# EspressoSystems/Push-CDN

Measured on AMD Instinct MI355X. Metric: broadcast_msgs_per_sec, higher is better.
Workload: dtype uint8; 1 GPU; model=gpu-broker-mesh, payload_bytes=1024, subscribers_total=10000, subscribers_per_broker=10000, topics=8, mode=broadcast, population=all, drops=0, parallelism=single-broker, global_batch=256, seq_len=1024

## Files before the change

csrc/common/tick_geom.h:

```cpp
#pragma once

#include <stdint.h>

#define K2B_BLK 32

#define DENSE_THREADS 256
#define DENSE_MAX_V 8
#define DENSE_GROUP 8
struct DenseGeom { int32_t n_chunks; int32_t chunk_units; };
static inline DenseGeom dense_geom(int32_t units_per_rec) {
    const int32_t cap = DENSE_THREADS * DENSE_MAX_V;
    const int32_t image = units_per_rec * K2B_BLK;
    DenseGeom g;
    g.n_chunks = (image + cap - 1) / cap;
    g.chunk_units = ((image + g.n_chunks - 1) / g.n_chunks + 63) & ~63;
    return g;
}
static inline int64_t dense_grid_x(int32_t n_users, int32_t group, int32_t n_chunks) {
    return ((int64_t)n_users + group - 1) / group * n_chunks;
}

static inline int64_t k2b_blocks(int64_t M) { return (M + K2B_BLK - 1) / K2B_BLK; }
static inline int64_t uniform_tick_scratch64(int64_t M, int64_t W, int64_t units_per_rec) {
    return 4 * M + W * M + k2b_blocks(M) * W * 64 + W * 64 + 2 * M * units_per_rec;
}
static inline int64_t uniform_tick_scratch32(int64_t M, int64_t W) {
    return 3 * M + 3 * k2b_blocks(M) * W * 64 + 2 * W * 64;
}

#define ROUTE_THREADS 256
struct RouteLds { int32_t mask, udst, ulim, usbase, pprefix, tslot, bcount, bytes; };
constexpr RouteLds route_lds(int32_t M) {
    const int32_t tiles = (M + K2B_BLK - 1) / K2B_BLK * 64;
    RouteLds l{};
    l.mask = 0;
    l.udst = l.mask + 8 * M;
    l.ulim = l.udst + 8 * 64;
    l.usbase = l.ulim + 4 * 64;
    l.pprefix = l.usbase + 4 * 64;
    l.tslot = l.pprefix + 2 * tiles;
    l.bcount = l.tslot + 2 * tiles;
    l.bytes = l.bcount + tiles;
    return l;
}
#define ROUTE_MAX_M 3584
static_assert(route_lds(ROUTE_MAX_M).bytes <= 64 * 1024, "route kernel LDS exceeds a workgroup's 64 KiB");
static_assert(route_lds(ROUTE_MAX_M + 1).bytes > 64 * 1024, "ROUTE_MAX_M is not the largest batch that fits");
static_assert(ROUTE_MAX_M >= 2048, "the 8-GPU bench routes 8 x 256 gathered messages per tick");
static_assert(ROUTE_MAX_M <= 65535 && K2B_BLK <= 255, "prefixes are 16-bit, tile counts 8-bit");
static_assert(route_lds(33).udst % 8 == 0 && route_lds(33).ulim % 4 == 0 && route_lds(33).pprefix % 2 == 0,
              "route kernel LDS arrays are aligned to their element types");
```

csrc/gpu_bindings.cpp:

```cpp

#include "binding_checks.h"
#include "hip/bls_kernels.h"
#include "hip/dataplane.h"

static inline void check_flat_shape(const torch::Tensor& pairs, int64_t units_per_pair) {
    TORCH_CHECK(units_per_pair >= 1 && units_per_pair <= (int64_t(1) << 21),
                "units_per_pair must be in [1, 2^21], got ", units_per_pair);
    TORCH_CHECK(pairs.size(0) * units_per_pair < (int64_t(1) << 31),
                "pair capacity * units_per_pair must be < 2^31, got ", pairs.size(0), " * ",
                units_per_pair);
}

std::vector<torch::Tensor> parse_batch(torch::Tensor buf, torch::Tensor offsets,
                                       uint64_t hash_seed) {
    Op a("parse_batch");
    const uint8_t* b = a.ptr<uint8_t>(buf, "buf");
    const int64_t* off = a.ptr<int64_t>(offsets, "offsets", 1);
    const int32_t M = a.i32(offsets.numel() - 1, "M");
    hipStream_t s = a.begin();
    auto o32 = opts(torch::kInt32, buf);
    auto o64 = opts(torch::kInt64, buf);
    auto disc = torch::empty({M}, o32);
    auto payload_off = torch::empty({M}, o64);
    auto payload_len = torch::empty({M}, o32);
// ... 485 lines not shown
}

void emit_direct_peers(torch::Tensor disc, torch::Tensor owner, torch::Tensor origin,
                       torch::Tensor payload_off, torch::Tensor payload_len,
                       int64_t ring_bytes, int64_t n_users, int64_t n_peers,
                       torch::Tensor ring_wpos, torch::Tensor n_pairs, torch::Tensor pairs,
                       torch::Tensor drops) {
    Op a("emit_direct_peers");
    const DirectArgs d = direct_args(a, disc, owner, payload_off, payload_len, ring_bytes);
    const int32_t* org = a.same<int32_t>(origin, "origin", d.M, "one per disc");
    const int32_t n = a.i32(n_users, "n_users");
    const int32_t p = a.i32(n_peers, "n_peers");
    uint64_t* wpos = a.ptr<uint64_t>(ring_wpos, "ring_wpos", int64_t(n) + p);
    int32_t* np = a.ptr<int32_t>(n_pairs, "n_pairs", 1);
    PairRec* pr = a.pairs(pairs);
    const int32_t capacity = a.i32(pairs.size(0), "pair capacity");
    uint32_t* dr = a.ptr<uint32_t>(drops, "drops", 1);
    hipStream_t s = a.begin();
    if (d.M == 0) return;
    launch_k5b_emit_direct_peers(d.disc, d.owner, org, d.payload_off, d.payload_len, d.M, n, p,
                                 ring_bytes, capacity, wpos, np, pr, dr, s);
    a.launched();
}

void direct_apply(torch::Tensor table_keys, torch::Tensor table_vals, torch::Tensor up_keys,
                  torch::Tensor up_owners, torch::Tensor del_keys, torch::Tensor n_failed) {
    Op a("direct_apply");
    uint64_t* keys = a.ptr<uint64_t>(table_keys, "table_keys", 1, vec());
    const int64_t S = table_keys.numel();
    TORCH_CHECK((S & (S - 1)) == 0, a.name(), ": table_keys must have a power-of-two length, got ",
                S);
    int32_t* vals = a.same<int32_t>(table_vals, "table_vals", S, "one per table_keys");
    const uint64_t* up = a.ptr<uint64_t>(up_keys, "up_keys");
    const int32_t n_up = a.i32(up_keys.numel(), "upsert count");
    const int32_t* owners = a.same<int32_t>(up_owners, "up_owners", n_up, "one per up_keys");
    const uint64_t* del = a.ptr<uint64_t>(del_keys, "del_keys");
    const int32_t n_del = a.i32(del_keys.numel(), "delete count");
    uint32_t* failed = a.ptr<uint32_t>(n_failed, "n_failed", 1);
    hipStream_t s = a.begin();
    launch_k6_direct_apply(keys, vals, S, up, owners, n_up, del, n_del, failed, s);
    a.launched();
}

void tick_uniform_broadcast(torch::Tensor buf, torch::Tensor offsets, uint64_t hash_seed,
                            torch::Tensor sub_bitmap, torch::Tensor ring_wpos,
                            int64_t ring_bytes, int64_t n_users, torch::Tensor pairs,
                            torch::Tensor drops, torch::Tensor n_pairs, torch::Tensor n_sparse,
                            torch::Tensor scratch64, torch::Tensor scratch32,
                            int64_t uniform_len, int64_t seq_base, torch::Tensor egress,
                            int64_t nt, int64_t dense) {
    Op a("tick_uniform_broadcast");
    UniformTick t;
    t.uniform_len = a.i32(uniform_len, "uniform_len", 0, (int64_t(1) << 30) - 1);
    const int64_t rec = (uniform_len + 16 + 15) & ~int64_t(15);
    t.rec = a.i32(rec, "rec");
    t.buf = a.ptr<uint8_t>(buf, "buf");
    t.offsets = a.ptr<int64_t>(offsets, "offsets", 1);
    const int64_t M = offsets.numel() - 1;
    t.M = a.i32(M, "M");
    t.hash_seed = hash_seed;
    t.sub_bitmap = a.ptr<uint64_t>(sub_bitmap, "sub_bitmap", 0, mat(256, -1));
    const int64_t W = sub_bitmap.size(1);
    t.W = a.i32(W, "W");
    t.n_users = a.i32(n_users, "n_users", 0, W * 64);
    a.ring_bytes(ring_bytes);
    t.ring_bytes = ring_bytes;
    t.ring_wpos = a.ptr<uint64_t>(ring_wpos, "ring_wpos", n_users);
    t.pairs = a.pairs(pairs);
    t.capacity = a.i32(pairs.size(0), "pair capacity");
    t.drops = a.ptr<uint32_t>(drops, "drops", 1);
    t.n_pairs = a.ptr<int32_t>(n_pairs, "n_pairs", 1);
    t.n_sparse = a.ptr<int32_t>(n_sparse, "n_sparse", 1);
    t.scratch64 = a.ptr<int64_t>(scratch64, "scratch64", uniform_tick_scratch64(M, W, rec / 16));
    t.scratch32 = a.ptr<int32_t>(scratch32, "scratch32", uniform_tick_scratch32(M, W));
    t.egress = a.ptr<uint8_t>(egress, "egress", n_users * ring_bytes);
    t.seq_base = (uint32_t)seq_base;
    t.nt = nt != 0;
    t.dense = dense != 0;
    TORCH_CHECK(buf.numel() >= M * uniform_len, a.name(), ": buf has ", buf.numel(),
                " bytes, shorter than M = ", M, " messages of uniform_len = ", uniform_len);
    check_flat_shape(pairs, rec / 16);
    TORCH_CHECK(M * (rec / 16) < (int64_t(1) << 31)
                && dense_grid_x(t.n_users, DENSE_GROUP, dense_geom((int32_t)(rec / 16)).n_chunks)
                       * k2b_blocks(M) < (int64_t(1) << 31),
                a.name(), ": batch too large for the dense fan-out");
    TORCH_CHECK((uintptr_t)t.scratch64 % 16 == 0, a.name(), ": scratch64 must be 16-byte aligned");
    hipStream_t s = a.begin();
    if (M == 0) return;
    launch_tick_uniform_broadcast(&t, s);
    a.launched();
}

std::vector<int64_t> uniform_tick_scratch_sizes(int64_t M, int64_t W, int64_t rec) {
    return {uniform_tick_scratch64(M, W, rec / 16), uniform_tick_scratch32(M, W)};
}

void drain_cursors(torch::Tensor ring_wpos, torch::Tensor staging, torch::Tensor host) {
    Op a("drain_cursors");
    int64_t* wpos = a.ptr<int64_t>(ring_wpos, "ring_wpos");
    const int32_t n = a.i32(ring_wpos.numel(), "cursor count");
    int64_t* st = a.ptr<int64_t>(staging, "staging", n);
    int64_t* h = a.ptr<int64_t>(host, "host", n, {}, Op::kPinnedHost);
    hipStream_t s = a.begin();
    if (n == 0) return;
    launch_drain_cursors(wpos, st, n, s);
    a.launched();
    a.check(hipMemcpyAsync(h, st, (size_t)n * 8, hipMemcpyDeviceToHost, s), "copy");
    a.check(hipStreamSynchronize(s), "sync");
}

PYBIND11_MODULE(TORCH_EXTENSION_NAME, m) {
    m.attr("_ROUTE_MAX_M") = py::int_(ROUTE_MAX_M);
    m.def("tick_uniform_broadcast", &tick_uniform_broadcast,
          "fused uniform broadcast tick: K4, K2a, K2b tiles, dense + sparse fan-out");
    m.def("uniform_tick_scratch_sizes", &uniform_tick_scratch_sizes,
          "(int64, int32) scratch elements tick_uniform_broadcast needs for (M, W, rec)");
    m.def("drain_cursors", &drain_cursors,
          "fused drain: cursors -> pinned host buffer, cursors zeroed, stream synchronised",
          py::call_guard<py::gil_scoped_release>());
    m.def("topic_mask_origin_t", &topic_mask_origin_t,
          "K2a transposed with per-message origin: remote-origin rows keep user bits only");
    m.def("emit_direct_peers", &emit_direct_peers,
          "K5b with peer recipient slots (owner -(p+2) -> ring n_users+p, local origin only)");
    m.def("direct_apply", &direct_apply,
          "K6: batched DirectMap upserts/deletes on the device table");
    m.def("parse_batch", &parse_batch, "K4: on-device capnp parse of a message batch",
          py::arg("buf"), py::arg("offsets"), py::arg("hash_seed") = 0);
    m.def("topic_mask", &topic_mask, "K2a: per-message subscriber mask");
    m.def("assign_emit", &assign_emit, "K2b: per-user FIFO ring assignment + pair list");
    m.def("fanout", &fanout, "K3: N-way payload fan-out into egress rings");
    m.def("direct_lookup", &direct_lookup, "K5: batched direct-route hash probe");
    m.def("apply_subs", &apply_subs, "K2c: apply subscribe/unsubscribe batch to bitmap");
    m.def("bls_verify_batch", &bls_verify_batch, "K1: batched BLS-over-BN254 verification");
    m.def("compact_rings", &compact_rings,
          "K7: gather used egress-ring prefixes into one staging buffer");
    m.def("precompute_g2_lines", &precompute_g2_lines,
          "fixed-g2 Miller line coefficients for K1 v2 (once per process)");
    m.def("bls_verify_batch2", &bls_verify_batch2,
          "K1 v2: 2-lane Fp2-decomposed batched BLS verification");
    m.def("bls_verify_batch_wave", &bls_verify_batch_wave,
          "K1 v3: wave-batched product verification (shared final exp, "
          "exact per-item fallback)");
    m.def("hash_to_g1_batch", &hash_to_g1_batch, "K1 helper: batched hash-to-G1");
    m.def("fanout_wave", &fanout_wave, "K3v2: wave-per-pair fan-out (nt flag, device count)");
    m.def("fanout_ref", &fanout_ref,
          "K3r: fan-out with by-reference records at or above ref_threshold");
    m.def("fanout_flat2", &fanout_flat2, "K3v4: flat fan-out, seq from base, capacity clamp");
    m.def("fanout_flat3", &fanout_flat3, "K3v5: graph-capturable (device seq counter)");
    m.def("seq_advance", &seq_advance, "bump the device seq counter (inside the graph)");
    m.def("topic_mask_t", &topic_mask_t, "K2a transposed: mask[W][M]");
    m.def("emit_direct", &emit_direct,
          "K5b: on-device direct-delivery pair emission (no host sync)");
    m.def("assign_emit_fused_t", &assign_emit_fused_t,
          "K2b fused on transposed mask (wave-aggregated claims, uniform-rec fast path)");
    m.def("assign_emit_blocks_t", &assign_emit_blocks_t,
          "K2b block-parallel (P1 count / P2 bases / P3 emit) for uniform records");
}
```

csrc/hip/dataplane.h:

```cpp
#pragma once

#include <hip/hip_runtime_api.h>
#include <stdint.h>

#include "../common/tick_geom.h"

struct alignas(16) PairRec { int32_t user; int32_t msg; int64_t dst; };
static_assert(sizeof(PairRec) == 16, "PairRec must be one dword4");

struct ParseOut {
    int32_t* disc;
    int64_t* payload_off;
    int32_t* payload_len;
    int64_t* topics_off;
    int32_t* topics_cnt;
    uint64_t* recip_hash;
    uint64_t* timestamp;
};

struct UniformTick {
    const uint8_t* buf;
    const int64_t* offsets;
    int32_t M;
    uint64_t hash_seed;
// ... 19 lines not shown

extern "C" {

void launch_k4_parse(const uint8_t* buf, const int64_t* offsets, int32_t M, uint64_t hash_seed,
                     ParseOut out, hipStream_t s);

void launch_k2a_topic_mask(const uint64_t* sub_bitmap, const uint8_t* buf,
                           const int64_t* topics_off, const int32_t* topics_cnt,
                           const int32_t* disc, uint64_t* mask, int32_t M, int32_t W,
                           hipStream_t s);
void launch_k2a_topic_mask_t(const uint64_t* sub_bitmap, const uint8_t* buf,
                             const int64_t* topics_off, const int32_t* topics_cnt,
                             const int32_t* disc, uint64_t* mask_t, int32_t M, int32_t W,
                             hipStream_t s);
void launch_k2a_topic_mask_origin_t(const uint64_t* sub_bitmap, const uint8_t* buf,
                                    const int64_t* topics_off, const int32_t* topics_cnt,
                                    const int32_t* disc, const int32_t* origin,
                                    uint64_t* mask_t, int32_t M, int32_t W, int32_t n_users,
                                    hipStream_t s);
void launch_k2c_apply_subs(uint64_t* sub_bitmap, const uint8_t* buf, const int64_t* topics_off,
                           const int32_t* topics_cnt, const int32_t* disc,
                           const int32_t* user_idx, int32_t M, int32_t W, hipStream_t s);

void launch_k2b_count(const uint64_t* mask, int32_t M, int32_t W, int32_t n_users,
                      int32_t* counts, hipStream_t s);
void launch_k2b_emit(const uint64_t* mask, const int64_t* payload_off,
                     const int32_t* payload_len, const int32_t* pair_base, int32_t M, int32_t W,
                     int32_t n_users, int64_t ring_bytes, uint64_t* ring_wpos, PairRec* pairs,
                     uint32_t* drops, hipStream_t s);
void launch_k2b_fused_t(const uint64_t* mask_t, const int32_t* payload_len, int32_t M,
                        int32_t W, int32_t n_users, int64_t ring_bytes, int32_t capacity,
                        int32_t uniform_rec, uint64_t* ring_wpos, int32_t* n_pairs,
                        PairRec* pairs, uint32_t* drops, hipStream_t s);
void launch_k2b_blocks_t(const uint64_t* mask_t, int32_t M, int32_t W, int32_t n_users,
                         int64_t ring_bytes, int32_t capacity, int32_t uniform_rec,
                         uint64_t* ring_wpos, int32_t* n_pairs, int32_t* bcount,
                         int32_t* pprefix, int32_t* ubase, int32_t* ufit, int64_t* udst,
                         PairRec* pairs, uint32_t* drops, hipStream_t s);

void launch_k3_fanout(const uint8_t* buf, const int64_t* payload_off,
                      const int32_t* payload_len, const PairRec* pairs, const uint32_t* msg_seq,
                      int32_t n_pairs, uint8_t* egress, hipStream_t s);
void launch_k3_fanout_wave(const uint8_t* buf, const int64_t* payload_off,
                           const int32_t* payload_len, const PairRec* pairs,
                           const uint32_t* msg_seq, const int32_t* n_pairs_ptr,
                           int32_t capacity, uint8_t* egress, int nt, int grid, hipStream_t s);
void launch_k3_fanout_ref(const uint8_t* buf, const int64_t* payload_off,
                          const int32_t* payload_len, const PairRec* pairs,
                          const uint32_t* msg_seq, const int32_t* n_pairs_ptr,
                          int32_t capacity, int32_t ref_threshold, int64_t ref_base,
                          uint8_t* egress, int nt, int grid, hipStream_t s);
void launch_k3_fanout_flat2(const uint8_t* buf, const int64_t* payload_off,
                            const int32_t* payload_len, const PairRec* pairs,
                            uint32_t seq_base, const int32_t* n_pairs_ptr, int32_t capacity,
                            int32_t units_per_pair, int32_t uniform_len, uint8_t* egress,
                            int nt, int grid, hipStream_t s);
void launch_k3_fanout_flat3(const uint8_t* buf, const int64_t* payload_off,
                            const int32_t* payload_len, const PairRec* pairs,
                            const uint32_t* seq_state, const int32_t* n_pairs_ptr,
                            int32_t capacity, int32_t units_per_pair, int32_t uniform_len,
                            uint8_t* egress, int nt, int grid, hipStream_t s);
void launch_k_seq_advance(uint32_t* seq_state, int32_t m, hipStream_t s);

void launch_k5_direct_lookup(const uint64_t* table_keys, const int32_t* table_vals,
                             int64_t table_size, const uint64_t* query, int32_t N,
                             int32_t* owner, hipStream_t s);
void launch_k5b_emit_direct(const int32_t* disc, const int32_t* owner,
                            const int64_t* payload_off, const int32_t* payload_len, int32_t M,
                            int64_t ring_bytes, int32_t capacity, uint64_t* ring_wpos,
                            int32_t* n_pairs, PairRec* pairs, uint32_t* drops, hipStream_t s);
void launch_k5b_emit_direct_peers(const int32_t* disc, const int32_t* owner,
                                  const int32_t* origin, const int64_t* payload_off,
                                  const int32_t* payload_len, int32_t M, int32_t n_users,
                                  int32_t n_peers, int64_t ring_bytes, int32_t capacity,
                                  uint64_t* ring_wpos, int32_t* n_pairs, PairRec* pairs,
                                  uint32_t* drops, hipStream_t s);
void launch_k6_direct_apply(uint64_t* table_keys, int32_t* table_vals, int64_t table_size,
                            const uint64_t* up_keys, const int32_t* up_owners, int32_t n_up,
                            const uint64_t* del_keys, int32_t n_del, uint32_t* n_failed,
                            hipStream_t s);

void launch_tick_uniform_broadcast(const UniformTick* t, hipStream_t s);

void launch_drain_cursors(int64_t* ring_wpos, int64_t* staging, int32_t n, hipStream_t s);

void launch_k7_compact_rings(const uint8_t* egress, int64_t ring_bytes, const int64_t* wpos,
                             const int64_t* dst_off, uint8_t* staging, int32_t n_rings,
                             int32_t max_chunks, hipStream_t s);

}
```

csrc/hip/dataplane.hip:

```cpp

#include <hip/hip_runtime.h>
#include <stdint.h>

#include "../common/divmagic.h"
#include "dataplane.h"

#define WAVE 64
#ifndef CDN_CHECK
#define CDN_CHECK 1
#endif

#define RING_ALIGN 16ull
__host__ __device__ inline uint64_t ring_rec(int32_t len) {
    return ((uint64_t)len + 16 + (RING_ALIGN - 1)) & ~(RING_ALIGN - 1);
}

typedef unsigned int cdn_v4u __attribute__((ext_vector_type(4)));
template <int NT>
__device__ __forceinline__ void store16(void* dst, cdn_v4u v) {
    if (NT) __builtin_nontemporal_store(v, (cdn_v4u*)dst);
    else *(cdn_v4u*)dst = v;
}

__device__ __forceinline__ void store_pair(PairRec* p, int32_t u, int32_t m, int64_t d) {
// ... 472 lines not shown
    const int64_t* __restrict__ payload_off,
    const int32_t* __restrict__ payload_len,
    const PairRec* __restrict__ pairs,
    const uint32_t* __restrict__ msg_seq,
    const int32_t* __restrict__ n_pairs_ptr,
    int32_t capacity,
    int32_t ref_threshold,
    int64_t ref_base,
    uint8_t* __restrict__ egress)
{
    int n_pairs = *n_pairs_ptr;
    if (n_pairs > capacity) n_pairs = capacity;
    const int lane = threadIdx.x & 63;
    const int wave_in_wg = threadIdx.x >> 6;
    const int waves_total = gridDim.x * 4;
    int gs = 0;
    while (gs < 6 && ((n_pairs - 1) >> gs) + 1 > waves_total) ++gs;
    const int n_groups = n_pairs > 0 ? ((n_pairs - 1) >> gs) + 1 : 0;
    for (int g = blockIdx.x * 4 + wave_in_wg; g < n_groups; g += waves_total) {
        const int64_t p = ((int64_t)g << gs) + lane;
        int32_t len = 0;
        uint32_t seq = 0;
        int64_t off = 0, dsto = 0;
        bool live = false;
        if (lane < (1 << gs) && p < n_pairs) {
            const PairRec pr = pairs[p];
            if (pr.user >= 0) {
                live = true;
                len = payload_len[pr.msg];
                off = payload_off[pr.msg];
                seq = msg_seq[pr.msg];
                dsto = pr.dst;
            }
        }
        const bool by_ref = live && len >= ref_threshold;
        if (by_ref) {
            const uint64_t ro = (uint64_t)(ref_base + off);
            store16<NT>(egress + dsto, cdn_v4u{(uint32_t)len | REF_FLAG, seq, (uint32_t)ro,
                                               (uint32_t)(ro >> 32)});
        }
        unsigned long long inl = __ballot(live && !by_ref);
        while (inl) {
            const int j = __ffsll((long long)inl) - 1;
            inl &= inl - 1;
            const int32_t jlen = __shfl(len, j);
            const uint32_t jseq = (uint32_t)__shfl((int)seq, j);
            const int64_t joff = ((int64_t)__shfl((int)(off >> 32), j) << 32)
                                 | (uint32_t)__shfl((int)off, j);
            const int64_t jdst = ((int64_t)__shfl((int)(dsto >> 32), j) << 32)
                                 | (uint32_t)__shfl((int)dsto, j);
            copy_record<NT>(egress + jdst, buf + joff, jlen, jseq, lane, WAVE);
        }
    }
}

extern "C" {

void launch_k3_fanout_ref(const uint8_t* buf, const int64_t* payload_off,
                          const int32_t* payload_len, const PairRec* pairs,
                          const uint32_t* msg_seq, const int32_t* n_pairs_ptr,
                          int32_t capacity, int32_t ref_threshold, int64_t ref_base,
                          uint8_t* egress, int nt, int grid, hipStream_t s) {
    if (grid <= 0) grid = 4096;
    DISPATCH_NT(nt, hipLaunchKernelGGL((k3_fanout_ref_t<NT>), dim3(grid), dim3(256), 0, s, buf,
                                       payload_off, payload_len, pairs, msg_seq, n_pairs_ptr,
                                       capacity, ref_threshold, ref_base, egress));
}

}

__device__ __forceinline__ cdn_v4u payload_unit(const uint8_t* __restrict__ msg, int32_t coff,
                                                int32_t len)
{
    const uint8_t* src = msg + coff;
    if (coff + 16 <= len && (((uintptr_t)src) & 15) == 0) return *(const cdn_v4u*)src;
    if (coff >= len) return cdn_v4u{0u, 0u, 0u, 0u};
    uint8_t tmp[16];
    #pragma unroll
    for (int b = 0; b < 16; ++b) tmp[b] = (coff + b < len) ? src[b] : 0;
    cdn_v4u v; memcpy(&v, tmp, 16);
    return v;
}

template <int NT, bool SEQ_FROM_PTR>
__global__ void __launch_bounds__(256) k3_fanout_flat_t(
    const uint8_t* __restrict__ buf,
    const int64_t* __restrict__ payload_off,
    const int32_t* __restrict__ payload_len,
    const PairRec* __restrict__ pairs,
    uint32_t seq_base_val,
    const uint32_t* __restrict__ seq_state,
    const int32_t* __restrict__ n_pairs_ptr,
    int32_t capacity,
    int32_t units_per_pair,
    uint32_t div_magic,
    int32_t div_shift,
    int32_t uniform_len,
    uint8_t* __restrict__ egress)
{
    const uint32_t seq_base = SEQ_FROM_PTR ? seq_state[0] : seq_base_val;
    int np = *n_pairs_ptr;
    if (np > capacity) np = capacity;
    const int64_t n_units = (int64_t)np * units_per_pair;
    const int64_t stride = (int64_t)gridDim.x * blockDim.x;
    for (int64_t f = (int64_t)blockIdx.x * blockDim.x + threadIdx.x; f < n_units; f += stride) {
        const uint32_t f32 = (uint32_t)f;
        const int p = (int)(((uint64_t)f32 * div_magic) >> div_shift);
        const int unit = (int)(f32 - (uint32_t)p * (uint32_t)units_per_pair);
        const PairRec pr = pairs[p];
        if (pr.user < 0) continue;
        const int mi = pr.msg;
        const int32_t len = uniform_len > 0 ? uniform_len : payload_len[mi];
        uint8_t* dst = egress + pr.dst + (size_t)unit * 16;
        if (unit == 0) {
            store16<NT>(dst, cdn_v4u{(uint32_t)len, seq_base + (uint32_t)mi, 0u, 0u});
            continue;
        }
        store16<NT>(dst, payload_unit(buf + payload_off[mi], (unit - 1) * 16, len));
    }
}


template <bool SEQ_FROM_PTR>
static void launch_flat(const uint8_t* buf, const int64_t* payload_off,
                        const int32_t* payload_len, const PairRec* pairs, uint32_t seq_base,
                        const uint32_t* seq_state, const int32_t* n_pairs_ptr, int32_t capacity,
                        int32_t units_per_pair, int32_t uniform_len, uint8_t* egress, int nt,
                        int grid, hipStream_t s) {
    if (grid <= 0) grid = 16384;
    uint32_t dm; int32_t dsh;
    u32_div_magic(units_per_pair, &dm, &dsh);
    DISPATCH_NT(nt, hipLaunchKernelGGL((k3_fanout_flat_t<NT, SEQ_FROM_PTR>), dim3(grid),
                                       dim3(256), 0, s, buf, payload_off, payload_len, pairs,
                                       seq_base, seq_state, n_pairs_ptr, capacity,
                                       units_per_pair, dm, dsh, uniform_len, egress));
}

extern "C" __global__ void k_seq_advance(uint32_t* seq_state, int32_t m) {
    if (blockIdx.x == 0 && threadIdx.x == 0) seq_state[0] += (uint32_t)m;
}

extern "C" {

void launch_k3_fanout_flat2(const uint8_t* buf, const int64_t* payload_off,
                            const int32_t* payload_len, const PairRec* pairs,
                            uint32_t seq_base, const int32_t* n_pairs_ptr, int32_t capacity,
                            int32_t units_per_pair, int32_t uniform_len, uint8_t* egress,
                            int nt, int grid, hipStream_t s) {
    launch_flat<false>(buf, payload_off, payload_len, pairs, seq_base, nullptr, n_pairs_ptr,
                       capacity, units_per_pair, uniform_len, egress, nt, grid, s);
}

void launch_k3_fanout_flat3(const uint8_t* buf, const int64_t* payload_off,
                            const int32_t* payload_len, const PairRec* pairs,
                            const uint32_t* seq_state, const int32_t* n_pairs_ptr,
                            int32_t capacity, int32_t units_per_pair, int32_t uniform_len,
                            uint8_t* egress, int nt, int grid, hipStream_t s) {
    launch_flat<true>(buf, payload_off, payload_len, pairs, 0u, seq_state, n_pairs_ptr,
                      capacity, units_per_pair, uniform_len, egress, nt, grid, s);
}

void launch_k_seq_advance(uint32_t* seq_state, int32_t m, hipStream_t s) {
    hipLaunchKernelGGL(k_seq_advance, dim3(1), dim3(1), 0, s, seq_state, m);
}

}

extern "C" __global__ void k2a_topic_mask_t(
    const uint64_t* __restrict__ sub_bitmap,
    const uint8_t* __restrict__ buf,
    const int64_t* __restrict__ topics_off,
    const int32_t* __restrict__ topics_cnt,
    const int32_t* __restrict__ disc,
    uint64_t* __restrict__ mask_t,
    int32_t M, int32_t W)
{
    int64_t idx = (int64_t)blockIdx.x * blockDim.x + threadIdx.x;
    if (idx >= (int64_t)M * W) return;
    int m = idx / W;
    int w = idx % W;
    mask_t[(int64_t)w * M + m] =
        topic_row_or<false>(sub_bitmap, buf, topics_off, topics_cnt, disc, m, w, W, nullptr, 0);
}

__device__ __forceinline__ int wave_claim_span(int count, int32_t* __restrict__ counter) {
    const int lane = threadIdx.x & 63;
    int incl = count;
    for (int d = 1; d < 64; d <<= 1) {
        int ngh = __shfl_up(incl, d);
        if (lane >= d) incl += ngh;
    }
    int wave_total = __shfl(incl, 63);
    int base = 0;
    if (lane == 0 && wave_total > 0) base = atomicAdd(counter, wave_total);
    base = __shfl(base, 0);
    return base + incl - count;
}

extern "C" __global__ void k2b_fused_t(
    const uint64_t* __restrict__ mask_t,
    const int32_t* __restrict__ payload_len,
    int32_t M, int32_t W, int32_t n_users,
// ... 598 lines not shown
extern "C" __global__ void __launch_bounds__(ROUTE_THREADS) k_route_word(
    const uint64_t* __restrict__ sub_bitmap,
    const uint8_t* __restrict__ buf,
    const int64_t* __restrict__ topics_off,
    const int32_t* __restrict__ topics_cnt,
    const int32_t* __restrict__ disc,
    int32_t M, int32_t W, int32_t NB, int32_t n_users,
    int64_t ring_bytes, int32_t capacity, int32_t uniform_rec, int32_t use_dense,
    uint64_t* __restrict__ ring_wpos,
    int32_t* __restrict__ n_pairs,
    int32_t* __restrict__ n_sparse,
    int64_t* __restrict__ tdst,
    PairRec* __restrict__ pairs,
    uint32_t* __restrict__ drops)
{
    extern __shared__ __attribute__((aligned(16))) uint8_t route_smem[];
    const RouteLds l = route_lds(M);
    uint64_t* wcol = (uint64_t*)(route_smem + l.mask);
    int64_t* udst = (int64_t*)(route_smem + l.udst);
    int32_t* ulim = (int32_t*)(route_smem + l.ulim);
    int32_t* usbase = (int32_t*)(route_smem + l.usbase);
    uint16_t* pprefix = (uint16_t*)(route_smem + l.pprefix);
    uint16_t* tslot = (uint16_t*)(route_smem + l.tslot);
    uint8_t* bcount = route_smem + l.bcount;

    const int w = blockIdx.x;
    const int lane = threadIdx.x & 63, wave = threadIdx.x >> 6, n_waves = blockDim.x >> 6;
    const int u = w * 64 + lane;

    for (int m = threadIdx.x; m < M; m += blockDim.x)
        wcol[m] = topic_row_or<false>(sub_bitmap, buf, topics_off, topics_cnt, disc, m, w, W,
                                      nullptr, 0);
    __syncthreads();
    for (int b = wave; b < NB; b += n_waves)
        bcount[b * 64 + lane] = (uint8_t)k2b_tile_count(wcol, M, b);
    __syncthreads();
    if (wave == 0) {
        const bool active = u < n_users;
        const K2bTiles r = k2b_tiles_body(bcount, u, active, 64, lane, M, W, NB, ring_bytes,
                                          capacity, uniform_rec, use_dense, ring_wpos, n_pairs,
                                          n_sparse, pprefix, tslot, tdst, drops);
        ulim[lane] = r.lim;
        usbase[lane] = r.sbase;
        udst[lane] = r.dst;
    }
    __syncthreads();
    for (int b = wave; b < NB; b += n_waves)
        k2b_p3_sparse_body(wcol, bcount, pprefix, tslot, tdst, ulim, usbase, udst, w, b, 64, lane,
                           M, W, n_users, uniform_rec, pairs);
}

__device__ __forceinline__ void k3d_image_body(
    const uint8_t* __restrict__ buf,
    const int64_t* __restrict__ offsets,
    int32_t M, int32_t units_per_rec, uint32_t div_magic, int32_t div_shift,
    int32_t uniform_len, uint32_t seq_base,
    cdn_v4u* __restrict__ image,
    uint32_t i)
{
    if (i >= (uint32_t)(M * units_per_rec)) return;
    const int m = (int)(((uint64_t)i * div_magic) >> div_shift);
    const int q = (int)i - m * units_per_rec;
    image[i] = q == 0 ? cdn_v4u{(uint32_t)uniform_len, seq_base + (uint32_t)m, 0u, 0u}
                      : payload_unit(buf + offsets[m], (q - 1) * 16, uniform_len);
}

extern "C" __global__ void __launch_bounds__(256) k_tick_prologue(
    const uint8_t* __restrict__ buf,
    const int64_t* __restrict__ offsets,
    int32_t M, uint64_t hash_seed, ParseOut out, int32_t parse_blocks,
    int32_t units_per_rec, uint32_t div_magic, int32_t div_shift,
    int32_t uniform_len, uint32_t seq_base,
    cdn_v4u* __restrict__ image,
    int32_t* __restrict__ n_pairs, int32_t* __restrict__ n_sparse)
{
    if (blockIdx.x == 0 && threadIdx.x == 0) { *n_pairs = 0; *n_sparse = 0; }
    if ((int32_t)blockIdx.x < parse_blocks)
        k4_parse_body(buf, offsets, M, hash_seed, out, blockIdx.x * blockDim.x + threadIdx.x);
    else
        k3d_image_body(buf, offsets, M, units_per_rec, div_magic, div_shift, uniform_len, seq_base,
                       image, (blockIdx.x - parse_blocks) * blockDim.x + threadIdx.x);
}

__global__ void __launch_bounds__(DENSE_THREADS) k3_fanout_dense(
    const cdn_v4u* __restrict__ image,
    const int64_t* __restrict__ tdst,
    int32_t M, int32_t NB, int32_t users64, int32_t n_users, int32_t units_per_rec,
    int32_t n_chunks, int32_t chunk_units, int32_t group,
    uint8_t* __restrict__ egress)
{
    const int per_group = NB * n_chunks;
    const int g = blockIdx.x / per_group, bc = blockIdx.x - g * per_group;
    const int b = bc / n_chunks, c = bc - b * n_chunks;
    const int m0 = b * K2B_BLK, nm = min(M - m0, K2B_BLK);
    const int lo = c * chunk_units + (int)threadIdx.x;
    const int hi = min(nm * units_per_rec, (c + 1) * chunk_units);
    if (lo >= hi) return;
    const cdn_v4u* __restrict__ img = image + (size_t)m0 * units_per_rec;
    cdn_v4u v[DENSE_MAX_V];
    #pragma unroll
    for (int k = 0; k < DENSE_MAX_V; ++k) {
        const int unit = lo + k * DENSE_THREADS;
        v[k] = unit < hi ? img[unit] : cdn_v4u{0u, 0u, 0u, 0u};
    }
    const int64_t* __restrict__ trow = tdst + (int64_t)b * users64;
    const int u1 = min(n_users, (g + 1) * group);
    for (int u = g * group; u < u1; ++u) {
        const int64_t d = trow[u];
        if (d < 0) continue;
        uint8_t* dst = egress + d + (size_t)lo * 16;
        #pragma unroll
        for (int k = 0; k < DENSE_MAX_V; ++k)
            if (lo + k * DENSE_THREADS < hi)
                store16<0>(dst + (size_t)k * (DENSE_THREADS * 16), v[k]);
    }
}

extern "C" __global__ void k_drain_cursors(int64_t* __restrict__ ring_wpos,
                                           int64_t* __restrict__ staging, int32_t n)
{
    const int i = blockIdx.x * blockDim.x + threadIdx.x;
    if (i >= n) return;
    staging[i] = ring_wpos[i];
    ring_wpos[i] = 0;
}

extern "C" {

void launch_tick_uniform_broadcast(const UniformTick* t, hipStream_t s) {
    const int32_t M = t->M, W = t->W;
    if (M <= 0) return;
    const int32_t NB = (int32_t)k2b_blocks(M);
    const int64_t U = (int64_t)W * 64, T = (int64_t)NB * U;
    const int32_t units = t->rec / 16;
    int64_t* p64 = t->scratch64;
    cdn_v4u* image = (cdn_v4u*)p64;  p64 += 2 * (int64_t)M * units;
    int64_t* payload_off = p64;  p64 += M;
    int64_t* topics_off = p64;   p64 += M;
    int64_t* recip_hash = p64;   p64 += M;
    int64_t* timestamp = p64;    p64 += M;
    uint64_t* mask_t = (uint64_t*)p64;  p64 += (int64_t)W * M;
    int64_t* tdst = p64;         p64 += T;
    int64_t* udst = p64;
    int32_t* p32 = t->scratch32;
    int32_t* disc = p32;         p32 += M;
    int32_t* payload_len = p32;  p32 += M;
    int32_t* topics_cnt = p32;   p32 += M;
    int32_t* bcount = p32;       p32 += T;
    int32_t* pprefix = p32;      p32 += T;
    int32_t* tslot = p32;        p32 += T;
    int32_t* ulim = p32;         p32 += U;
    int32_t* usbase = p32;

    const int threads = 256;
    const int parse_blocks = (M + threads - 1) / threads;
    const int image_blocks = t->dense ? (M * units + threads - 1) / threads : 0;
    uint32_t dm; int32_t dsh;
    u32_div_magic(units, &dm, &dsh);
    hipLaunchKernelGGL(k_tick_prologue, dim3(parse_blocks + image_blocks), dim3(threads), 0, s,
                       t->buf, t->offsets, M, t->hash_seed,
                       ParseOut{disc, payload_off, payload_len, topics_off, topics_cnt,
                                (uint64_t*)recip_hash, (uint64_t*)timestamp},
                       parse_blocks, units, dm, dsh, t->uniform_len, t->seq_base, image,
                       t->n_pairs, t->n_sparse);

    if (M <= ROUTE_MAX_M) {
        hipLaunchKernelGGL(k_route_word, dim3(W), dim3(ROUTE_THREADS), route_lds(M).bytes, s,
                           t->sub_bitmap, t->buf, topics_off, topics_cnt, disc, M, W, NB,
                           t->n_users, t->ring_bytes, t->capacity, t->rec, t->dense ? 1 : 0,
                           t->ring_wpos, t->n_pairs, t->n_sparse, tdst, t->pairs, t->drops);
    } else {
        launch_k2a_topic_mask_t(t->sub_bitmap, t->buf, topics_off, topics_cnt, disc, mask_t, M, W,
                                s);
        const int blocks_wb = (W * NB * 64 + threads - 1) / threads;
        const int blocks_u = (t->n_users + threads - 1) / threads;
        hipLaunchKernelGGL(k2b_p1_count_z, dim3(blocks_wb), dim3(threads), 0, s, mask_t, M, W, NB,
                           bcount, t->n_pairs, t->n_sparse);
        hipLaunchKernelGGL(k2b_p2_tiles, dim3(blocks_u), dim3(threads), 0, s, bcount, M, W, NB,
                           t->n_users, t->ring_bytes, t->capacity, t->rec, t->dense ? 1 : 0,
                           t->ring_wpos, t->n_pairs, t->n_sparse, pprefix, tslot, tdst, ulim,
                           usbase, udst, t->drops);
        hipLaunchKernelGGL(k2b_p3_sparse, dim3(blocks_wb), dim3(threads), 0, s, mask_t, bcount,
                           pprefix, tslot, tdst, ulim, usbase, udst, M, W, NB, t->n_users, t->rec,
                           t->pairs);
    }

    if (t->dense) {
        const DenseGeom geo = dense_geom(units);
        const dim3 grid((uint32_t)(dense_grid_x(t->n_users, DENSE_GROUP, geo.n_chunks) * NB));
        hipLaunchKernelGGL(k3_fanout_dense, grid, dim3(DENSE_THREADS), 0, s, image, tdst, M, NB,
                           (int32_t)U, t->n_users, units, geo.n_chunks, geo.chunk_units,
                           DENSE_GROUP, t->egress);
    }
    launch_flat<false>(t->buf, t->offsets, payload_len, t->pairs, t->seq_base, nullptr,
                       t->n_sparse, t->capacity, units, t->uniform_len, t->egress, t->nt, 0, s);
}

void launch_drain_cursors(int64_t* ring_wpos, int64_t* staging, int32_t n, hipStream_t s) {
    if (n <= 0) return;
    hipLaunchKernelGGL(k_drain_cursors, dim3((n + 255) / 256), dim3(256), 0, s, ring_wpos,
                       staging, n);
}

}
```

pushcdn_amd/broker/gpu_engine.py:

```python

from __future__ import annotations

import os

from dataclasses import dataclass
from typing import Dict, List, Optional, Tuple

import torch

from ..utils.keyhash import fnv1a64
from ..utils.log import get_logger

log = get_logger("gpu-engine")

RING_ALIGN = 16
REF_FLAG = 0x80000000


def ring_rec(length: int) -> int:
    return (length + 16 + (RING_ALIGN - 1)) & ~(RING_ALIGN - 1)


@dataclass
class TickStats:
# ... 24 lines not shown
    ) -> None:
        assert n_peer_slots >= 0
        self.n_peer_slots = n_peer_slots
        self.n_recipients = n_users + n_peer_slots
        self.pair_capacity = pair_capacity
        self._flat_max_rec = int(os.environ.get("PUSHCDN_FLAT_MAX_REC", "4096"))
        flat_units = self._flat_max_rec // 16 + 1
        assert 1 <= flat_units <= (1 << 21), "PUSHCDN_FLAT_MAX_REC too large"
        assert pair_capacity * flat_units < (1 << 31), (
            f"pair_capacity {pair_capacity} x {flat_units} flat units/record "
            "must stay below 2^31")
        self.nt_fanout = nt_fanout
        self.direct_enabled = direct_enabled
        self.fused_tick = fused_tick
        self.fused_ticks = 0
        self.hash_seed = hash_seed & ((1 << 64) - 1)
        self.fanout_wire = fanout_wire
        self.device = torch.device(device)
        self.is_cuda = self.device.type == "cuda"
        if use_gpu_ops is None:
            use_gpu_ops = self.is_cuda
        self.use_gpu_ops = use_gpu_ops
        if self.use_gpu_ops:
            from ..ops import get_gpu_ops

            self._ops = get_gpu_ops()
        else:
            self._ops = None

        assert ring_bytes % 16 == 0
        self.n_users = n_users
        self.ring_bytes = ring_bytes
        R = self.n_recipients
        self.W = (R + 63) // 64

        dev = self.device
        self.sub_bitmap = torch.zeros((256, self.W), dtype=torch.int64, device=dev)
        self.egress = torch.zeros(R * ring_bytes, dtype=torch.uint8, device=dev)
        self.ring_wpos = torch.zeros(R, dtype=torch.int64, device=dev)
        self.direct_keys = torch.zeros(direct_table_size, dtype=torch.int64, device=dev)
        self.direct_vals = torch.zeros(direct_table_size, dtype=torch.int32, device=dev)
        self._direct_entries: Dict[int, int] = {}
        self._direct_pubkeys: Dict[int, bytes] = {}
        self._direct_tombstones: set = set()
        self._direct_failed = torch.zeros(1, dtype=torch.int32, device=dev)
        self._mship_rows: Dict[int, list] = {}
        self._mship_direct: Dict[int, Tuple[Optional[int], bool]] = {}
        self._ctl_ops = None
        if ref_threshold is not None:
            assert fanout_wire, "ref_threshold requires fanout_wire=True"
            assert 1 <= ref_threshold < REF_FLAG
            assert ring_rec(ref_threshold - 1) <= ring_bytes, (
                f"ref_threshold {ref_threshold}: an inline message just below it "
                f"does not fit a {ring_bytes}-byte ring")
        self.ref_threshold = ref_threshold
        self._ref_batches: List[bytes] = []
        self._ref_base = 0
        self.loss_accounting = loss_accounting
        self._acct_ops = None
        self._losses: Dict[int, int] = {}
        if loss_accounting:
            self.demand = torch.zeros(R, dtype=torch.int64, device=dev)
            if self.use_gpu_ops:
                from ..ops import get_gpu_acct_ops

                self._acct_ops = get_gpu_acct_ops()
                self._lossy = torch.empty((max(R, 1), 2), dtype=torch.int64, device=dev)
                self._n_lossy = torch.zeros(1, dtype=torch.int32, device=dev)
                self._n_lossy_host = torch.zeros(1, dtype=torch.int32,
                                                 pin_memory=self.is_cuda)
        self.seq = 0
        self.total = TickStats()
        self._staging_dev: Optional[torch.Tensor] = None
        self._staging_host: Optional[torch.Tensor] = None
        if self.use_gpu_ops:
            o32 = dict(dtype=torch.int32, device=dev)
            self._pairs = torch.empty((pair_capacity, 4), **o32)
            self._drops = torch.zeros(1, **o32)
            self._n_pairs = torch.zeros(1, **o32)
            self._seq_dev = torch.zeros(1, **o32)
            self._n_sparse = torch.zeros(1, **o32)
            self._dense_fanout = True
            self._fused_scratch = None
            self._drain_bufs = None
            self._graphs: Dict[Tuple[int, int, int], object] = {}


    def subscribe(self, user_idx: int, topics: List[int]) -> None:
        self.flush_membership()
        w, bit = user_idx >> 6, 1 << (user_idx & 63)
        bit = bit - (1 << 64) if bit >= (1 << 63) else bit
        for t in topics:
            self.sub_bitmap[t & 0xFF, w] |= bit

    def unsubscribe(self, user_idx: int, topics: List[int]) -> None:
        self.flush_membership()
        w, bit = user_idx >> 6, 1 << (user_idx & 63)
        bit = bit - (1 << 64) if bit >= (1 << 63) else bit
        for t in topics:
            self.sub_bitmap[t & 0xFF, w] &= ~bit

    def subscribe_all(self, topics: List[int]) -> None:
        self.flush_membership()
        if self.n_peer_slots:
            full = self._user_bit_words().to(self.device)
            for t in topics:
                self.sub_bitmap[t & 0xFF] |= full
            return
        full = torch.full((self.W,), -1, dtype=torch.int64)
        tail = self.n_users & 63
        if tail:
            full[-1] = (1 << tail) - 1
        for t in topics:
            self.sub_bitmap[t & 0xFF] = full.to(self.device)

    def _user_bit_words(self) -> torch.Tensor:
        words = torch.zeros(self.W, dtype=torch.int64)
        nfull = self.n_users >> 6
        words[:nfull] = -1
        tail = self.n_users & 63
        if tail:
            words[nfull] = (1 << tail) - 1
        return words


    def _peer_word_bit(self, p: int) -> Tuple[int, int]:
        if not 0 <= p < self.n_peer_slots:
            raise IndexError(f"peer slot {p} outside [0, {self.n_peer_slots})")
        r = self.n_users + p
        bit = 1 << (r & 63)
        return r >> 6, (bit - (1 << 64) if bit >= (1 << 63) else bit)

    def set_peer_topics(self, p: int, topics: List[int]) -> None:
        self.flush_membership()
        w, bit = self._peer_word_bit(p)
        self.sub_bitmap[:, w] &= ~bit
        rows = sorted({t & 0xFF for t in topics})
        if rows:
            self.sub_bitmap[torch.tensor(rows, device=self.device), w] |= bit

    def clear_peer(self, p: int) -> None:
        self.flush_membership()
        w, bit = self._peer_word_bit(p)
        self.sub_bitmap[:, w] &= ~bit
        self.ring_wpos[self.n_users + p] = 0
        if self.loss_accounting:
            self.demand[self.n_users + p] = 0

    def _direct_hash(self, pubkey: bytes) -> int:
        h = fnv1a64(pubkey, self.hash_seed)
        prev = self._direct_pubkeys.get(h)
        if prev is not None and prev != pubkey:
            raise ValueError("direct routing-hash collision; refusing registration")
        return h

    def register_direct(self, pubkey: bytes, owner: int) -> None:
        self.flush_membership()
        h = self._direct_hash(pubkey)
        self._direct_pubkeys[h] = pubkey
        self._direct_entries[h] = owner
        self._rebuild_direct_table()

    def register_direct_bulk(self, entries) -> None:
        self.flush_membership()
        for pubkey, owner in entries:
            h = self._direct_hash(pubkey)
# ... 229 lines not shown
        host = torch.frombuffer(bytearray(batch), dtype=torch.uint8)
        off = torch.tensor(offsets, dtype=torch.int64)
        if staging is not None:
            assert staging.numel() >= host.numel()
            dst = staging[:host.numel()]
            dst.copy_(host, non_blocking=self.is_cuda)
            if self.is_cuda:
                return dst, off.to(self.device, non_blocking=True)
            return dst, off
        if self.is_cuda:
            return host.to(self.device, non_blocking=True), off.to(self.device, non_blocking=True)
        return host, off

    def tick(self, buf: torch.Tensor, offsets: torch.Tensor,
             host_batch: Optional[bytes] = None,
             host_offsets: Optional[List[int]] = None,
             uniform_wire_len: Optional[int] = None,
             origin=None) -> TickStats:
        self.flush_membership()
        ref_base = 0
        if self.ref_threshold is not None:
            if host_batch is None or host_offsets is None:
                raise ValueError("by-reference delivery needs host_batch and host_offsets")
            ref_base = self._retain_batch(host_batch, host_offsets)
        if self.use_gpu_ops:
            return self._tick_gpu(buf, offsets, uniform_wire_len, origin, ref_base)
        assert host_batch is not None and host_offsets is not None
        return self._tick_cpu(host_batch, host_offsets, origin, ref_base)

    def _retain_batch(self, host_batch, host_offsets) -> int:
        thr = self.ref_threshold
        base = self._ref_base
        if any(host_offsets[i + 1] - host_offsets[i] >= thr
               for i in range(len(host_offsets) - 1)):
            self._ref_batches.append(host_batch)
            self._ref_base = base + len(host_batch)
        return base

    def _discard_ref_batches(self) -> None:
        self._ref_batches = []
        self._ref_base = 0

    def _k2b_block_scratch(self, M: int):
        NB = (M + 31) // 32
        W64 = self.W * 64
        cur = getattr(self, "_k2b_scratch", None)
        if cur is not None and cur[0] >= NB:
            return cur[1]
        o32 = dict(dtype=torch.int32, device=self.device)
        bufs = (
            torch.empty(NB * W64, **o32),
            torch.empty(NB * W64, **o32),
            torch.empty(W64, **o32),
            torch.empty(W64, **o32),
            torch.empty(W64, dtype=torch.int64, device=self.device),
        )
        self._k2b_scratch = (NB, bufs)
        return bufs

    def _assign_emit(self, ops, mask_t, payload_len, rec: int, M: int) -> None:
        if rec and self.use_gpu_ops:
            bcount, pprefix, ubase, ufit, udst = self._k2b_block_scratch(M)
            ops.assign_emit_blocks_t(
                mask_t, self.ring_wpos, self.ring_bytes, self.n_recipients,
                bcount, pprefix, ubase, ufit, udst,
                self._pairs, self._drops, self._n_pairs, rec,
            )
        else:
            ops.assign_emit_fused_t(
                mask_t, payload_len, self.ring_wpos, self.ring_bytes, self.n_recipients,
                self._pairs, self._drops, self._n_pairs, rec,
            )

    def _fused_tick_ok(self, uniform_wire_len: Optional[int], origin) -> bool:
        return (self.fused_tick and not self.loss_accounting
                and self.fanout_wire and uniform_wire_len is not None
                and not self.direct_enabled and self.n_peer_slots == 0
                and origin is None and self.ref_threshold is None
                and ring_rec(uniform_wire_len) <= self._flat_max_rec)

    def _tick_fused(self, buf: torch.Tensor, offsets: torch.Tensor,
                    uniform_wire_len: int, M: int) -> TickStats:
        ops = self._ops
        n64, n32 = ops.uniform_tick_scratch_sizes(M, self.W, ring_rec(uniform_wire_len))
        s64, s32 = self._fused_scratch or (None, None)
        if s64 is None or s64.numel() < n64 or s32.numel() < n32:
            s64 = torch.empty(max(n64, 0 if s64 is None else s64.numel()),
                              dtype=torch.int64, device=self.device)
            s32 = torch.empty(max(n32, 0 if s32 is None else s32.numel()),
                              dtype=torch.int32, device=self.device)
            self._fused_scratch = (s64, s32)
        seq_base = self.seq
        self.seq += M
        ops.tick_uniform_broadcast(
            buf, offsets, self.hash_seed, self.sub_bitmap, self.ring_wpos, self.ring_bytes,
            self.n_recipients, self._pairs, self._drops, self._n_pairs, self._n_sparse,
            s64, s32, uniform_wire_len, seq_base, self.egress,
            1 if self.nt_fanout else 0, 1 if self._dense_fanout else 0)
        self.fused_ticks += 1
        return TickStats(n_messages=M)

    def _tick_gpu(self, buf: torch.Tensor, offsets: torch.Tensor,
                  uniform_wire_len: Optional[int] = None, origin=None,
                  ref_base: int = 0) -> TickStats:
        ops = self._ops
        M = offsets.shape[0] - 1
        if M > 0 and self._fused_tick_ok(uniform_wire_len, origin):
            return self._tick_fused(buf, offsets, uniform_wire_len, M)
        disc, payload_off, payload_len, topics_off, topics_cnt, recip_hash, _ts = ops.parse_batch(
            buf, offsets, self.hash_seed
        )
        peer_plane = self.n_peer_slots > 0 or origin is not None
        if peer_plane:
            origin = self._origin_tensor(origin, M)
            mask_t = ops.topic_mask_origin_t(self.sub_bitmap, buf, topics_off, topics_cnt,
                                             disc, origin, self.n_users)
        else:
            mask_t = ops.topic_mask_t(self.sub_bitmap, buf, topics_off, topics_cnt, disc)
        if self.fanout_wire:
            payload_off = offsets[:-1].contiguous()
            payload_len = (offsets[1:] - offsets[:-1]).to(torch.int32).contiguous()
        self._n_pairs.zero_()
        uniform = self.fanout_wire and uniform_wire_len is not None
        thr = self.ref_threshold
        ring_len = payload_len
        if thr is not None:
            if uniform and uniform_wire_len >= thr:
                uniform = False
            if not uniform:
                ring_len = torch.where(payload_len >= thr, 0, payload_len).to(torch.int32)
        rec = ring_rec(uniform_wire_len) if uniform else 0
        self._assign_emit(ops, mask_t, ring_len, rec, M)
        owner = None
        if self.direct_enabled:
            owner = ops.direct_lookup(self.direct_keys, self.direct_vals, recip_hash)
            if peer_plane:
                ops.emit_direct_peers(disc, owner, origin, payload_off, ring_len,
                                      self.ring_bytes, self.n_users, self.n_peer_slots,
                                      self.ring_wpos, self._n_pairs, self._pairs,
                                      self._drops)
            else:
                ops.emit_direct(disc, owner, payload_off, ring_len, self.ring_bytes,
                                self.ring_wpos, self._n_pairs, self._pairs, self._drops)
        if self._acct_ops is not None and M > 0:
            self._acct_ops.recipient_demand(
                self.demand, mask_t, ring_len.contiguous(), disc, owner,
                origin if peer_plane else None, self.n_users, self.n_peer_slots)
        seq_base = self.seq
        self.seq += M
        nt = 1 if self.nt_fanout else 0
        if uniform and rec <= self._flat_max_rec:
            units = rec // 16
            ops.fanout_flat2(buf, payload_off, payload_len, self._pairs, seq_base,
                             self._n_pairs, units, self.egress, nt, 0,
                             uniform_wire_len)
        else:
            seq = torch.arange(seq_base, seq_base + M, dtype=torch.int32, device=self.device)
            if thr is not None:
                ops.fanout_ref(buf, payload_off, payload_len, self._pairs, seq,
                               self._n_pairs, self.egress, nt, 0, thr, ref_base)
            else:
                ops.fanout_wave(buf, payload_off, payload_len, self._pairs, seq,
                                self._n_pairs, self.egress, nt, 0)
        return TickStats(n_messages=M)

    def _graph_tick_body(self, buf: torch.Tensor, offsets: torch.Tensor, units: int) -> None:
        ops = self._ops
        M = offsets.shape[0] - 1
        disc, _po, _pl, topics_off, topics_cnt, _rh, _ts = ops.parse_batch(
            buf, offsets, self.hash_seed
        )
        mask_t = ops.topic_mask_t(self.sub_bitmap, buf, topics_off, topics_cnt, disc)
        payload_off = offsets[:-1].contiguous()
        payload_len = (offsets[1:] - offsets[:-1]).to(torch.int32).contiguous()
# ... 229 lines not shown
```

Before: 443,200 msgs/s.

## Fuse sparse flat fan-out into dense kernel tail, zero-copy cursor drain

```diff
diff --git a/csrc/common/tick_geom.h b/csrc/common/tick_geom.h
--- a/csrc/common/tick_geom.h
+++ b/csrc/common/tick_geom.h
@@ -19,6 +19,8 @@
 static inline int64_t dense_grid_x(int32_t n_users, int32_t group, int32_t n_chunks) {
     return ((int64_t)n_users + group - 1) / group * n_chunks;
 }
+
+#define SPARSE_TAIL_BLOCKS 16384
 
 static inline int64_t k2b_blocks(int64_t M) { return (M + K2B_BLK - 1) / K2B_BLK; }
 static inline int64_t uniform_tick_scratch64(int64_t M, int64_t W, int64_t units_per_rec) {
diff --git a/csrc/gpu_bindings.cpp b/csrc/gpu_bindings.cpp
--- a/csrc/gpu_bindings.cpp
+++ b/csrc/gpu_bindings.cpp
@@ -591,7 +591,7 @@
     check_flat_shape(pairs, rec / 16);
     TORCH_CHECK(M * (rec / 16) < (int64_t(1) << 31)
                 && dense_grid_x(t.n_users, DENSE_GROUP, dense_geom((int32_t)(rec / 16)).n_chunks)
-                       * k2b_blocks(M) < (int64_t(1) << 31),
+                       * k2b_blocks(M) + SPARSE_TAIL_BLOCKS < (int64_t(1) << 31),
                 a.name(), ": batch too large for the dense fan-out");
     TORCH_CHECK((uintptr_t)t.scratch64 % 16 == 0, a.name(), ": scratch64 must be 16-byte aligned");
     hipStream_t s = a.begin();
@@ -612,14 +612,22 @@
     int64_t* h = a.ptr<int64_t>(host, "host", n, {}, Op::kPinnedHost);
     hipStream_t s = a.begin();
     if (n == 0) return;
-    launch_drain_cursors(wpos, st, n, s);
-    a.launched();
-    a.check(hipMemcpyAsync(h, st, (size_t)n * 8, hipMemcpyDeviceToHost, s), "copy");
+    void* h_dev = nullptr;
+    if (hipHostGetDevicePointer(&h_dev, h, 0) == hipSuccess && h_dev != nullptr) {
+        launch_drain_cursors(wpos, (int64_t*)h_dev, n, s);
+        a.launched();
+    } else {
+        (void)hipGetLastError();
+        launch_drain_cursors(wpos, st, n, s);
+        a.launched();
+        a.check(hipMemcpyAsync(h, st, (size_t)n * 8, hipMemcpyDeviceToHost, s), "copy");
+    }
     a.check(hipStreamSynchronize(s), "sync");
 }
 
 PYBIND11_MODULE(TORCH_EXTENSION_NAME, m) {
     m.attr("_ROUTE_MAX_M") = py::int_(ROUTE_MAX_M);
+    m.attr("_SPARSE_TAIL_BLOCKS") = py::int_(SPARSE_TAIL_BLOCKS);
     m.def("tick_uniform_broadcast", &tick_uniform_broadcast,
           "fused uniform broadcast tick: K4, K2a, K2b tiles, dense + sparse fan-out");
     m.def("uniform_tick_scratch_sizes", &uniform_tick_scratch_sizes,
diff --git a/csrc/hip/dataplane.h b/csrc/hip/dataplane.h
--- a/csrc/hip/dataplane.h
+++ b/csrc/hip/dataplane.h
@@ -125,7 +125,7 @@
 
 void launch_tick_uniform_broadcast(const UniformTick* t, hipStream_t s);
 
-void launch_drain_cursors(int64_t* ring_wpos, int64_t* staging, int32_t n, hipStream_t s);
+void launch_drain_cursors(int64_t* ring_wpos, int64_t* out, int32_t n, hipStream_t s);
 
 void launch_k7_compact_rings(const uint8_t* egress, int64_t ring_bytes, const int64_t* wpos,
                              const int64_t* dst_off, uint8_t* staging, int32_t n_rings,
diff --git a/csrc/hip/dataplane.hip b/csrc/hip/dataplane.hip
--- a/csrc/hip/dataplane.hip
+++ b/csrc/hip/dataplane.hip
@@ -578,28 +578,27 @@
     return v;
 }
 
-template <int NT, bool SEQ_FROM_PTR>
-__global__ void __launch_bounds__(256) k3_fanout_flat_t(
+template <int NT>
+__device__ __forceinline__ void k3_flat_body(
     const uint8_t* __restrict__ buf,
     const int64_t* __restrict__ payload_off,
     const int32_t* __restrict__ payload_len,
     const PairRec* __restrict__ pairs,
-    uint32_t seq_base_val,
-    const uint32_t* __restrict__ seq_state,
+    uint32_t seq_base,
     const int32_t* __restrict__ n_pairs_ptr,
     int32_t capacity,
     int32_t units_per_pair,
     uint32_t div_magic,
     int32_t div_shift,
     int32_t uniform_len,
-    uint8_t* __restrict__ egress)
-{
-    const uint32_t seq_base = SEQ_FROM_PTR ? seq_state[0] : seq_base_val;
+    uint8_t* __restrict__ egress,
+    uint32_t block, uint32_t n_blocks)
+{
     int np = *n_pairs_ptr;
     if (np > capacity) np = capacity;
     const int64_t n_units = (int64_t)np * units_per_pair;
-    const int64_t stride = (int64_t)gridDim.x * blockDim.x;
-    for (int64_t f = (int64_t)blockIdx.x * blockDim.x + threadIdx.x; f < n_units; f += stride) {
+    const int64_t stride = (int64_t)n_blocks * blockDim.x;
+    for (int64_t f = (int64_t)block * blockDim.x + threadIdx.x; f < n_units; f += stride) {
         const uint32_t f32 = (uint32_t)f;
         const int p = (int)(((uint64_t)f32 * div_magic) >> div_shift);
         const int unit = (int)(f32 - (uint32_t)p * (uint32_t)units_per_pair);
@@ -614,6 +613,27 @@
         }
         store16<NT>(dst, payload_unit(buf + payload_off[mi], (unit - 1) * 16, len));
     }
+}
+
+template <int NT, bool SEQ_FROM_PTR>
+__global__ void __launch_bounds__(256) k3_fanout_flat_t(
+    const uint8_t* __restrict__ buf,
+    const int64_t* __restrict__ payload_off,
+    const int32_t* __restrict__ payload_len,
+    const PairRec* __restrict__ pairs,
+    uint32_t seq_base_val,
+    const uint32_t* __restrict__ seq_state,
+    const int32_t* __restrict__ n_pairs_ptr,
+    int32_t capacity,
+    int32_t units_per_pair,
+    uint32_t div_magic, int32_t div_shift,
+    int32_t uniform_len,
+    uint8_t* __restrict__ egress)
+{
+    const uint32_t seq_base = SEQ_FROM_PTR ? seq_state[0] : seq_base_val;
+    k3_flat_body<NT>(buf, payload_off, payload_len, pairs, seq_base, n_pairs_ptr, capacity,
+                     units_per_pair, div_magic, div_shift, uniform_len, egress, blockIdx.x,
+                     gridDim.x);
 }
 
 
@@ -1378,15 +1398,15 @@
                        image, (blockIdx.x - parse_blocks) * blockDim.x + threadIdx.x);
 }
 
-__global__ void __launch_bounds__(DENSE_THREADS) k3_fanout_dense(
+__device__ __forceinline__ void k3_dense_body(
     const cdn_v4u* __restrict__ image,
     const int64_t* __restrict__ tdst,
     int32_t M, int32_t NB, int32_t users64, int32_t n_users, int32_t units_per_rec,
     int32_t n_chunks, int32_t chunk_units, int32_t group,
-    uint8_t* __restrict__ egress)
+    uint8_t* __restrict__ egress, uint32_t block)
 {
     const int per_group = NB * n_chunks;
-    const int g = blockIdx.x / per_group, bc = blockIdx.x - g * per_group;
+    const int g = block / per_group, bc = block - g * per_group;
     const int b = bc / n_chunks, c = bc - b * n_chunks;
     const int m0 = b * K2B_BLK, nm = min(M - m0, K2B_BLK);
     const int lo = c * chunk_units + (int)threadIdx.x;
@@ -1412,12 +1432,37 @@
     }
 }
 
+static_assert(DENSE_THREADS == 256, "the tail runs the flat body, 256 threads per workgroup");
+template <int NT>
+__global__ void __launch_bounds__(DENSE_THREADS) k3_fanout_dense_tail_t(
+    const cdn_v4u* __restrict__ image,
+    const int64_t* __restrict__ tdst,
+    int32_t M, int32_t NB, int32_t users64, int32_t n_users, int32_t units_per_rec,
+    int32_t n_chunks, int32_t chunk_units, int32_t group, uint32_t dense_blocks,
+    const uint8_t* __restrict__ buf,
+    const int64_t* __restrict__ offsets,
+    const int32_t* __restrict__ payload_len,
+    const PairRec* __restrict__ pairs,
+    uint32_t seq_base,
+    const int32_t* __restrict__ n_sparse,
+    int32_t capacity, uint32_t div_magic, int32_t div_shift, int32_t uniform_len,
+    uint8_t* __restrict__ egress)
+{
+    if (blockIdx.x < dense_blocks)
+        k3_dense_body(image, tdst, M, NB, users64, n_users, units_per_rec, n_chunks, chunk_units,
+                      group, egress, blockIdx.x);
+    else
+        k3_flat_body<NT>(buf, offsets, payload_len, pairs, seq_base, n_sparse, capacity,
+                         units_per_rec, div_magic, div_shift, uniform_len, egress,
+                         blockIdx.x - dense_blocks, gridDim.x - dense_blocks);
+}
+
 extern "C" __global__ void k_drain_cursors(int64_t* __restrict__ ring_wpos,
-                                           int64_t* __restrict__ staging, int32_t n)
+                                           int64_t* __restrict__ out, int32_t n)
 {
     const int i = blockIdx.x * blockDim.x + threadIdx.x;
     if (i >= n) return;
-    staging[i] = ring_wpos[i];
+    out[i] = ring_wpos[i];
     ring_wpos[i] = 0;
 }
 
@@ -1483,19 +1528,25 @@
 
     if (t->dense) {
         const DenseGeom geo = dense_geom(units);
-        const dim3 grid((uint32_t)(dense_grid_x(t->n_users, DENSE_GROUP, geo.n_chunks) * NB));
-        hipLaunchKernelGGL(k3_fanout_dense, grid, dim3(DENSE_THREADS), 0, s, image, tdst, M, NB,
-                           (int32_t)U, t->n_users, units, geo.n_chunks, geo.chunk_units,
-                           DENSE_GROUP, t->egress);
-    }
-    launch_flat<false>(t->buf, t->offsets, payload_len, t->pairs, t->seq_base, nullptr,
-                       t->n_sparse, t->capacity, units, t->uniform_len, t->egress, t->nt, 0, s);
-}
-
-void launch_drain_cursors(int64_t* ring_wpos, int64_t* staging, int32_t n, hipStream_t s) {
+        const uint32_t dense_blocks =
+            (uint32_t)(dense_grid_x(t->n_users, DENSE_GROUP, geo.n_chunks) * NB);
+        DISPATCH_NT(t->nt, hipLaunchKernelGGL(
+            (k3_fanout_dense_tail_t<NT>), dim3(dense_blocks + SPARSE_TAIL_BLOCKS),
+            dim3(DENSE_THREADS), 0, s, image, tdst, M, NB, (int32_t)U, t->n_users, units,
+            geo.n_chunks, geo.chunk_units, DENSE_GROUP, dense_blocks, t->buf, t->offsets,
+            payload_len, t->pairs, t->seq_base, t->n_sparse, t->capacity, dm, dsh,
+            t->uniform_len, t->egress));
+    } else {
+        launch_flat<false>(t->buf, t->offsets, payload_len, t->pairs, t->seq_base, nullptr,
+                           t->n_sparse, t->capacity, units, t->uniform_len, t->egress, t->nt, 0,
+                           s);
+    }
+}
+
+void launch_drain_cursors(int64_t* ring_wpos, int64_t* out, int32_t n, hipStream_t s) {
     if (n <= 0) return;
-    hipLaunchKernelGGL(k_drain_cursors, dim3((n + 255) / 256), dim3(256), 0, s, ring_wpos,
-                       staging, n);
-}
-
-}
+    hipLaunchKernelGGL(k_drain_cursors, dim3((n + 255) / 256), dim3(256), 0, s, ring_wpos, out,
+                       n);
+}
+
+}
diff --git a/pushcdn_amd/broker/gpu_engine.py b/pushcdn_amd/broker/gpu_engine.py
--- a/pushcdn_amd/broker/gpu_engine.py
+++ b/pushcdn_amd/broker/gpu_engine.py
@@ -130,6 +130,7 @@
             self._n_sparse = torch.zeros(1, **o32)
             self._dense_fanout = True
             self._fused_scratch = None
+            self._fused_scratch_shape = None
             self._drain_bufs = None
             self._graphs: Dict[Tuple[int, int, int], object] = {}
 
@@ -525,14 +526,17 @@
     def _tick_fused(self, buf: torch.Tensor, offsets: torch.Tensor,
                     uniform_wire_len: int, M: int) -> TickStats:
         ops = self._ops
-        n64, n32 = ops.uniform_tick_scratch_sizes(M, self.W, ring_rec(uniform_wire_len))
+        shape = (M, self.W, uniform_wire_len)
         s64, s32 = self._fused_scratch or (None, None)
-        if s64 is None or s64.numel() < n64 or s32.numel() < n32:
-            s64 = torch.empty(max(n64, 0 if s64 is None else s64.numel()),
-                              dtype=torch.int64, device=self.device)
-            s32 = torch.empty(max(n32, 0 if s32 is None else s32.numel()),
-                              dtype=torch.int32, device=self.device)
-            self._fused_scratch = (s64, s32)
+        if shape != self._fused_scratch_shape:
+            n64, n32 = ops.uniform_tick_scratch_sizes(M, self.W, ring_rec(uniform_wire_len))
+            if s64 is None or s64.numel() < n64 or s32.numel() < n32:
+                s64 = torch.empty(max(n64, 0 if s64 is None else s64.numel()),
+                                  dtype=torch.int64, device=self.device)
+                s32 = torch.empty(max(n32, 0 if s32 is None else s32.numel()),
+                                  dtype=torch.int32, device=self.device)
+                self._fused_scratch = (s64, s32)
+            self._fused_scratch_shape = shape
         seq_base = self.seq
         self.seq += M
         ops.tick_uniform_broadcast(
```

Measured after the change: 452,300 msgs/s, median of 6. 1.02x the previous value.
